# sdwyc/ROLO

Hardware: AMD Instinct MI355X
Metric: scans/sec (128k-pt frame, 20 GN iters) (higher is better)
Workload: dtype f64

## Files before the change

### rolo_amd/csrc/dev_math.hpp

```cpp
#pragma once
#include <hip/hip_runtime.h>

#define ROLO_DEV __device__ __forceinline__

namespace rolo {

ROLO_DEV int f2ord(float f) { int i = __float_as_int(f); return i >= 0 ? i : i ^ 0x7fffffff; }
ROLO_DEV float ord2f(int k) { int i = k >= 0 ? k : k ^ 0x7fffffff; return __int_as_float(i); }


struct Sym3 { double xx, xy, xz, yy, yz, zz; };
struct Vec3 { double x, y, z; };
struct Mat3 { double m[9]; };

ROLO_DEV Vec3 mat3_mulv(const double* R, const Vec3& p) {
  return Vec3{R[0] * p.x + R[1] * p.y + R[2] * p.z, R[3] * p.x + R[4] * p.y + R[5] * p.z, R[6] * p.x + R[7] * p.y + R[8] * p.z};
}

ROLO_DEV Sym3 sym3_rotate(const double* R, const Sym3& C) {
  double a00 = R[0] * C.xx + R[1] * C.xy + R[2] * C.xz, a01 = R[0] * C.xy + R[1] * C.yy + R[2] * C.yz, a02 = R[0] * C.xz + R[1] * C.yz + R[2] * C.zz;
  double a10 = R[3] * C.xx + R[4] * C.xy + R[5] * C.xz, a11 = R[3] * C.xy + R[4] * C.yy + R[5] * C.yz, a12 = R[3] * C.xz + R[4] * C.yz + R[5] * C.zz;
  double a20 = R[6] * C.xx + R[7] * C.xy + R[8] * C.xz, a21 = R[6] * C.xy + R[7] * C.yy + R[8] * C.yz, a22 = R[6] * C.xz + R[7] * C.yz + R[8] * C.zz;
  Sym3 o;
  o.xx = a00 * R[0] + a01 * R[1] + a02 * R[2];
  o.xy = a00 * R[3] + a01 * R[4] + a02 * R[5];
  o.xz = a00 * R[6] + a01 * R[7] + a02 * R[8];
  o.yy = a10 * R[3] + a11 * R[4] + a12 * R[5];
  o.yz = a10 * R[6] + a11 * R[7] + a12 * R[8];
  o.zz = a20 * R[6] + a21 * R[7] + a22 * R[8];
  return o;
}

ROLO_DEV Sym3 sym3_add(const Sym3& a, const Sym3& b) { return Sym3{a.xx + b.xx, a.xy + b.xy, a.xz + b.xz, a.yy + b.yy, a.yz + b.yz, a.zz + b.zz}; }

ROLO_DEV Sym3 sym3_inverse(const Sym3& A) {
  double c00 = A.yy * A.zz - A.yz * A.yz;
  double c01 = A.xz * A.yz - A.xy * A.zz;
  double c02 = A.xy * A.yz - A.xz * A.yy;
  double c11 = A.xx * A.zz - A.xz * A.xz;
  double c12 = A.xz * A.xy - A.xx * A.yz;
  double c22 = A.xx * A.yy - A.xy * A.xy;
  double det = A.xx * c00 + A.xy * c01 + A.xz * c02;
  double inv = 1.0 / det;
  return Sym3{c00 * inv, c01 * inv, c02 * inv, c11 * inv, c12 * inv, c22 * inv};
}

ROLO_DEV Vec3 sym3_mulv(const Sym3& M, const Vec3& e) {
  return Vec3{M.xx * e.x + M.xy * e.y + M.xz * e.z, M.xy * e.x + M.yy * e.y + M.yz * e.z, M.xz * e.x + M.yz * e.y + M.zz * e.z};
}
ROLO_DEV double dot3(const Vec3& a, const Vec3& b) { return a.x * b.x + a.y * b.y + a.z * b.z; }

template <int OFF>
ROLO_DEV int lane_xor_b32(int x) {
  if constexpr (OFF == 32) {
    const auto r = __builtin_amdgcn_permlane32_swap((unsigned)x, (unsigned)x, false, false);
    return (int)((threadIdx.x & 32) ? r[0] : r[1]);
  } else if constexpr (OFF == 16) {
    const auto r = __builtin_amdgcn_permlane16_swap((unsigned)x, (unsigned)x, false, false);
    return (int)((threadIdx.x & 16) ? r[0] : r[1]);
  } else if constexpr (OFF == 8) {
    return __builtin_amdgcn_update_dpp(0, x, 0x128, 0xf, 0xf, false);
  } else if constexpr (OFF == 4) {
    const int a = __builtin_amdgcn_update_dpp(0, x, 0x104, 0xf, 0x5, false);
    return __builtin_amdgcn_update_dpp(a, x, 0x114, 0xf, 0xa, false);
  } else if constexpr (OFF == 2) {
    return __builtin_amdgcn_update_dpp(0, x, 0x4E, 0xf, 0xf, false);
  } else {
    return __builtin_amdgcn_update_dpp(0, x, 0xB1, 0xf, 0xf, false);
  }
}
template <int OFF>
ROLO_DEV double lane_xor_f64(double v) {
  return __hiloint2double(lane_xor_b32<OFF>(__double2hiint(v)), lane_xor_b32<OFF>(__double2loint(v)));
}

template <int OFF>
ROLO_DEV unsigned long long lane_xor_u64(unsigned long long v) {
  const unsigned lo = (unsigned)lane_xor_b32<OFF>((int)(unsigned)(v & 0xffffffffull)), hi = (unsigned)lane_xor_b32<OFF>((int)(unsigned)(v >> 32));
  return ((unsigned long long)hi << 32) | lo;
}

}
```

### rolo_amd/csrc/knn_cov.hip

```cpp
#include <cstdio>
#include <cstring>
#include <string.h>
#include "rolo_internal.hpp"
#include "switches.hpp"
#include "dev_math.hpp"
#include "voxel_dev.hpp"
#ifdef ROLO_KNN_ROCPRIM_SORT
#include <rocprim/rocprim.hpp>
#endif
#include <cfloat>
#include <climits>

namespace rolo {

namespace {


constexpr int BBOX_BLOCKS = 128;
constexpr int BBOX_PART = 16;

__global__ __launch_bounds__(256) void bbox_kernel(KnnPair A, int* bbox) {
  __shared__ float smn[4][3], smx[4][3];
  const int which = blockIdx.x / BBOX_BLOCKS, blk = blockIdx.x - which * BBOX_BLOCKS;
  const float4* __restrict__ p = A.c[which].xyz;
// ... 263 lines not shown
  if (g < P && s < n) {
    const uint32_t idx = order[s];
    const float4 q = p[idx];
    o = make_float4(q.x, q.y, q.z, __int_as_float((int)idx));
  }
  if (g >= P) return;
  const bool real = __float_as_int(o.w) != INT_MAX;
  float lox = real ? o.x : INFINITY, loy = real ? o.y : INFINITY, loz = real ? o.z : INFINITY;
  float hix = real ? o.x : -INFINITY, hiy = real ? o.y : -INFINITY, hiz = real ? o.z : -INFINITY;
  if (g < n_leaves) sorted[s] = o;
#pragma unroll
  for (int m = 1; m < KNN_LEAF; m <<= 1) {
    lox = fminf(lox, __shfl_xor(lox, m)); loy = fminf(loy, __shfl_xor(loy, m)); loz = fminf(loz, __shfl_xor(loz, m));
    hix = fmaxf(hix, __shfl_xor(hix, m)); hiy = fmaxf(hiy, __shfl_xor(hiy, m)); hiz = fmaxf(hiz, __shfl_xor(hiz, m));
  }
  if ((s & (KNN_LEAF - 1)) == 0) {
    boxes[2 * (size_t)(P + g)] = make_float4(lox, loy, loz, 0.f);
    boxes[2 * (size_t)(P + g) + 1] = make_float4(hix, hiy, hiz, 0.f);
  }
  constexpr int LPB = 256 / KNN_LEAF;
  if (P >= LPB) {
    __shared__ float4 nlo[LPB], nhi[LPB];
    const int lt = threadIdx.x / KNN_LEAF;
    if ((s & (KNN_LEAF - 1)) == 0) { nlo[lt] = make_float4(lox, loy, loz, 0.f); nhi[lt] = make_float4(hix, hiy, hiz, 0.f); }
    __syncthreads();
    const size_t g0 = (size_t)P + (size_t)(g - lt);
    int m = LPB; size_t first = g0;
    while (m > 1) {
      const int half = m >> 1;
      first >>= 1;
      float4 a, b;
      const int u = threadIdx.x;
      if (u < half) {
        const float4 l0 = nlo[2 * u], l1 = nlo[2 * u + 1], h0 = nhi[2 * u], h1 = nhi[2 * u + 1];
        a = make_float4(fminf(l0.x, l1.x), fminf(l0.y, l1.y), fminf(l0.z, l1.z), 0.f);
        b = make_float4(fmaxf(h0.x, h1.x), fmaxf(h0.y, h1.y), fmaxf(h0.z, h1.z), 0.f);
      }
      __syncthreads();
      if (u < half) { nlo[u] = a; nhi[u] = b; boxes[2 * (first + u)] = a; boxes[2 * (first + u) + 1] = b; }
      __syncthreads();
      m = half;
    }
  }
}

__global__ __launch_bounds__(256) void tree_reduce_kernel(float4* boxes0, int count_in0, int chunk0, int split, float4* boxes1, int count_in1, int chunk1) {
  ROLO_ALL_KERNEL_PRIO();
  __shared__ float4 lo[512], hi[512];
  const bool second = (int)blockIdx.x >= split;
  float4* boxes = second ? boxes1 : boxes0;
  const int count_in = second ? count_in1 : count_in0, chunk = second ? chunk1 : chunk0;
  const int b = (int)blockIdx.x - (second ? split : 0), t = threadIdx.x;
  const size_t base_in = (size_t)count_in + (size_t)b * chunk;
  for (int i = t; i < chunk; i += 256) { lo[i] = boxes[2 * (base_in + i)]; hi[i] = boxes[2 * (base_in + i) + 1]; }
  __syncthreads();
  int m = chunk, level_count = count_in;
  while (m > 1) {
    const int half = m >> 1;
    level_count >>= 1;
    float4 nlo, nhi;
    if (t < half) {
      float4 a = lo[2 * t], c = lo[2 * t + 1], e = hi[2 * t], f = hi[2 * t + 1];
      nlo = make_float4(fminf(a.x, c.x), fminf(a.y, c.y), fminf(a.z, c.z), 0.f);
      nhi = make_float4(fmaxf(e.x, f.x), fmaxf(e.y, f.y), fmaxf(e.z, f.z), 0.f);
    }
    __syncthreads();
    if (t < half) {
      lo[t] = nlo; hi[t] = nhi;
      size_t h = (size_t)level_count + (size_t)b * half + t;
      boxes[2 * h] = nlo; boxes[2 * h + 1] = nhi;
    }
    __syncthreads();
    m = half;
  }
}

struct Rot2 { double c, s; };

ROLO_DEV void make_jacobi(double x, double y, double z, Rot2& r) {
  double deno = 2.0 * fabs(y);
  if (deno < DBL_MIN) { r.c = 1; r.s = 0; return; }
  double tau = (x - z) / deno;
  double w = sqrt(tau * tau + 1.0);
  double t = (tau > 0) ? 1.0 / (tau + w) : 1.0 / (tau - w);
  double sign_t = t > 0 ? 1.0 : -1.0;
  double n = 1.0 / sqrt(t * t + 1.0);
  r.s = -sign_t * (y / fabs(y)) * fabs(t) * n;
  r.c = n;
}

template <int P_, int Q_>
ROLO_DEV bool jacobi_pair(double (&W)[9], double (&U)[9], double (&V)[9], double& max_diag) {
  const double threshold = fmax(DBL_MIN, 2.0 * DBL_EPSILON * max_diag);
  if (!(fabs(W[P_ * 3 + Q_]) > threshold || fabs(W[Q_ * 3 + P_]) > threshold)) return false;
  double m00 = W[P_ * 3 + P_], m01 = W[P_ * 3 + Q_], m10 = W[Q_ * 3 + P_], m11 = W[Q_ * 3 + Q_];
  Rot2 rot1;
  double t = m00 + m11, d = m10 - m01;
  if (fabs(d) < DBL_MIN) { rot1.s = 0; rot1.c = 1; }
  else { double u = t / d; double tmp = sqrt(1.0 + u * u); rot1.s = 1.0 / tmp; rot1.c = u / tmp; }
  double n00 = rot1.c * m00 + rot1.s * m10, n01 = rot1.c * m01 + rot1.s * m11, n11 = -rot1.s * m01 + rot1.c * m11;
  Rot2 jr; make_jacobi(n00, n01, n11, jr);
  Rot2 jl; { double c2 = jr.c, s2 = -jr.s; jl.c = rot1.c * c2 - rot1.s * s2; jl.s = rot1.c * s2 + rot1.s * c2; }
#pragma unroll
  for (int k = 0; k < 3; k++) { double x = W[P_ * 3 + k], y = W[Q_ * 3 + k]; W[P_ * 3 + k] = jl.c * x + jl.s * y; W[Q_ * 3 + k] = -jl.s * x + jl.c * y; }
#pragma unroll
  for (int k = 0; k < 3; k++) { double x = U[k * 3 + P_], y = U[k * 3 + Q_]; U[k * 3 + P_] = jl.c * x + jl.s * y; U[k * 3 + Q_] = -jl.s * x + jl.c * y; }
#pragma unroll
  for (int k = 0; k < 3; k++) { double x = W[k * 3 + P_], y = W[k * 3 + Q_]; W[k * 3 + P_] = jr.c * x - jr.s * y; W[k * 3 + Q_] = jr.s * x + jr.c * y; }
#pragma unroll
  for (int k = 0; k < 3; k++) { double x = V[k * 3 + P_], y = V[k * 3 + Q_]; V[k * 3 + P_] = jr.c * x - jr.s * y; V[k * 3 + Q_] = jr.s * x + jr.c * y; }
  max_diag = fmax(max_diag, fmax(fabs(W[P_ * 3 + P_]), fabs(W[Q_ * 3 + Q_])));
  return true;
}

ROLO_DEV void swap_cols(double (&M)[9], int a, int b) {
#pragma unroll
  for (int k = 0; k < 3; k++) { double t = M[k * 3 + a]; M[k * 3 + a] = M[k * 3 + b]; M[k * 3 + b] = t; }
}

ROLO_DEV void jacobi_svd3(const double (&A)[9], double (&U)[9], double (&sv)[3], double (&V)[9]) {
  double scale = 0;
#pragma unroll
  for (int i = 0; i < 9; i++) scale = fmax(scale, fabs(A[i]));
  if (!(scale > 0) || !isfinite(scale)) scale = 1.0;
  double W[9];
#pragma unroll
  for (int i = 0; i < 9; i++) { W[i] = A[i] / scale; U[i] = (i % 4 == 0) ? 1.0 : 0.0; V[i] = (i % 4 == 0) ? 1.0 : 0.0; }
  double max_diag = fmax(fabs(W[0]), fmax(fabs(W[4]), fabs(W[8])));
  for (int sweep = 0; sweep < 100; sweep++) {
    bool any = false;
    any |= jacobi_pair<1, 0>(W, U, V, max_diag);
    any |= jacobi_pair<2, 0>(W, U, V, max_diag);
    any |= jacobi_pair<2, 1>(W, U, V, max_diag);
    if (!any) break;
  }
#pragma unroll
  for (int i = 0; i < 3; i++) {
    double a = fabs(W[i * 4]);
    sv[i] = a * scale;
    if (a != 0) { double sgn = W[i * 4] / a; U[0 * 3 + i] *= sgn; U[1 * 3 + i] *= sgn; U[2 * 3 + i] *= sgn; }
  }
  if (sv[1] > sv[0] && sv[1] >= sv[2]) { double t = sv[0]; sv[0] = sv[1]; sv[1] = t; swap_cols(U, 0, 1); swap_cols(V, 0, 1); }
  else if (sv[2] > sv[0] && sv[2] > sv[1]) { double t = sv[0]; sv[0] = sv[2]; sv[2] = t; swap_cols(U, 0, 2); swap_cols(V, 0, 2); }
  if (sv[2] > sv[1]) { double t = sv[1]; sv[1] = sv[2]; sv[2] = t; swap_cols(U, 1, 2); swap_cols(V, 1, 2); }
}

ROLO_DEV void inv3(const double (&A)[9], double (&o)[9]) {
  double c00 = A[4] * A[8] - A[5] * A[7], c01 = A[2] * A[7] - A[1] * A[8], c02 = A[1] * A[5] - A[2] * A[4];
  double c10 = A[5] * A[6] - A[3] * A[8], c11 = A[0] * A[8] - A[2] * A[6], c12 = A[2] * A[3] - A[0] * A[5];
  double c20 = A[3] * A[7] - A[4] * A[6], c21 = A[1] * A[6] - A[0] * A[7], c22 = A[0] * A[4] - A[1] * A[3];
  double det = A[0] * c00 + A[1] * c10 + A[2] * c20;
  double inv = 1.0 / det;
  o[0] = c00 * inv; o[1] = c01 * inv; o[2] = c02 * inv; o[3] = c10 * inv; o[4] = c11 * inv; o[5] = c12 * inv; o[6] = c20 * inv; o[7] = c21 * inv; o[8] = c22 * inv;
}

ROLO_DEV void knn_covariance_finish(double cxx, double cxy, double cxz, double cyy, double cyz, double czz, int n, int qi, int reg,
                                    double* __restrict__ cov, double (&c6)[6], double* __restrict__ nrm = nullptr) {
  double out[9];

  if (reg == ROLO_REG_NONE) {
    out[0] = cxx; out[1] = cxy; out[2] = cxz; out[3] = cxy; out[4] = cyy; out[5] = cyz; out[6] = cxz; out[7] = cyz; out[8] = czz;
  } else if (reg == ROLO_REG_FROBENIUS) {
    double C[9] = {cxx + 1e-3, cxy, cxz, cxy, cyy + 1e-3, cyz, cxz, cyz, czz + 1e-3};
    double Ci[9]; inv3(C, Ci);
    double nrm = 0;
#pragma unroll
    for (int i = 0; i < 9; i++) nrm += Ci[i] * Ci[i];
    nrm = sqrt(nrm);
#pragma unroll
    for (int i = 0; i < 9; i++) Ci[i] /= nrm;
    inv3(Ci, out);
  } else {
    const double A[9] = {cxx, cxy, cxz, cxy, cyy, cyz, cxz, cyz, czz};
    double U[9], V[9], sv[3];
    jacobi_svd3(A, U, sv, V);
    double v0 = 1, v1 = 1, v2 = 1e-3;
    if (reg == ROLO_REG_MIN_EIG) { v0 = fmax(sv[0], 1e-3); v1 = fmax(sv[1], 1e-3); v2 = fmax(sv[2], 1e-3); }
    else if (reg == ROLO_REG_NORMALIZED_MIN_EIG) { double m = fmax(sv[0], fmax(sv[1], sv[2])); v0 = fmax(sv[0] / m, 1e-3); v1 = fmax(sv[1] / m, 1e-3); v2 = fmax(sv[2] / m, 1e-3); }
    else if (reg == ROLO_REG_PLANE_S) { double s = sv[0] + sv[1] + sv[2]; v0 = sv[0] / s; v1 = sv[1] / s; v2 = 1e-3; }
#pragma unroll
    for (int a = 0; a < 3; a++)
#pragma unroll
      for (int b = 0; b < 3; b++) out[a * 3 + b] = (U[a * 3 + 0] * v0) * V[b * 3 + 0] + (U[a * 3 + 1] * v1) * V[b * 3 + 1] + (U[a * 3 + 2] * v2) * V[b * 3 + 2];
    if (nrm && reg == ROLO_REG_PLANE) {
      const double s3 = U[0 * 3 + 2] * V[0 * 3 + 2] + U[1 * 3 + 2] * V[1 * 3 + 2] + U[2 * 3 + 2] * V[2 * 3 + 2];
      const double al = sqrt(1.0 - (s3 < 0 ? -1e-3 : 1e-3));
      const double s1 = U[0 * 3 + 0] * V[0 * 3 + 0] + U[1 * 3 + 0] * V[1 * 3 + 0] + U[2 * 3 + 0] * V[2 * 3 + 0];
      const double s2 = U[0 * 3 + 1] * V[0 * 3 + 1] + U[1 * 3 + 1] * V[1 * 3 + 1] + U[2 * 3 + 1] * V[2 * 3 + 1];
      const bool plane_form = s1 > 0 && s2 > 0;
      const size_t pn = (size_t)n;
      nrm[qi] = plane_form ? al * V[0 * 3 + 2] : __builtin_nan(""); nrm[pn + qi] = al * V[1 * 3 + 2]; nrm[2 * pn + qi] = al * V[2 * 3 + 2];
    }
  }
  const size_t pitch = (size_t)n;
  c6[0] = out[0]; c6[1] = 0.5 * (out[1] + out[3]); c6[2] = 0.5 * (out[2] + out[6]); c6[3] = out[4]; c6[4] = 0.5 * (out[5] + out[7]); c6[5] = out[8];
#pragma unroll
  for (int d = 0; d < 6; d++) cov[d * pitch + qi] = c6[d];
}

template <int KMAX>
ROLO_DEV void knn_neighbourhood_moments(const int (&ki)[KMAX], int kk, const float4* __restrict__ orig, double (&m6)[6]) {
  float px[KMAX], py[KMAX], pz[KMAX];
#pragma unroll
  for (int u = 0; u < KMAX; u++) {
    const float4 p = (u < kk) ? orig[ki[u]] : make_float4(0.f, 0.f, 0.f, 0.f);
    px[u] = p.x; py[u] = p.y; pz[u] = p.z;
  }
  double mx = 0, my = 0, mz = 0;
#pragma unroll
  for (int u = 0; u < KMAX; u++) if (u < kk) { mx += (double)px[u]; my += (double)py[u]; mz += (double)pz[u]; }
  mx /= kk; my /= kk; mz /= kk;
  double cxx = 0, cxy = 0, cxz = 0, cyy = 0, cyz = 0, czz = 0;
#pragma unroll
  for (int u = 0; u < KMAX; u++) if (u < kk) {
    const double ax = (double)px[u] - mx, ay = (double)py[u] - my, az = (double)pz[u] - mz;
    cxx += ax * ax; cxy += ax * ay; cxz += ax * az; cyy += ay * ay; cyz += ay * az; czz += az * az;
  }
  m6[0] = cxx / kk; m6[1] = cxy / kk; m6[2] = cxz / kk; m6[3] = cyy / kk; m6[4] = cyz / kk; m6[5] = czz / kk;
}

template <int KMAX>
ROLO_DEV void knn_covariance_tail(const int (&ki)[KMAX], int kk, const float4* __restrict__ orig, int n, int qi, int reg,
                                  double* __restrict__ cov, double (&c6)[6], double* __restrict__ nrm = nullptr) {
// ... 27 lines not shown
#ifdef ROLO_KNN_ROCPRIM_SORT
  return false;
#else
  return true;
#endif
}

size_t knn_bbox_ints() { return BBOX_PART + 2 * BBOX_BLOCKS * 6; }

size_t knn_sort_temp_bytes(int n) {
#ifdef ROLO_KNN_ROCPRIM_SORT
  size_t bytes = 0;
  (void)rocprim::radix_sort_pairs(nullptr, bytes, (uint32_t*)nullptr, (uint32_t*)nullptr, (uint32_t*)nullptr, (uint32_t*)nullptr,
                                  (size_t)n, 0, 31, (hipStream_t)0);
  return bytes;
#else
  (void)n;
  return sizeof(int) * SORT_PASSES * SORT_NB * SORT_D;
#endif
}

hipError_t launch_knn_build(const KnnPair& A_in, void* sort_tmp, size_t sort_tmp_bytes, uint32_t* keys0, uint32_t* keys1,
                            uint32_t* vals0, uint32_t* vals1, int* bbox, const VoxelFuse& vf, hipStream_t s) {
  KnnPair A = A_in;
  bool have_parts = true;
  for (int i = 0; i < A.n_clouds; i++) have_parts = have_parts && A.c[i].bpart != nullptr && A.c[i].n_bpart > 0;
  if (!have_parts) for (int i = 0; i < A.n_clouds; i++) { A.c[i].bpart = bbox + BBOX_PART + i * BBOX_BLOCKS * 6; A.c[i].n_bpart = BBOX_BLOCKS; }
  const int nc = A.n_clouds;
  const int n_total = A.c[0].n + (nc > 1 ? A.c[1].n : 0);
#ifdef ROLO_KNN_ROCPRIM_SORT
  const int tile_ = ((n_total + SORT_NB - 1) / SORT_NB + SORT_T - 1) / SORT_T * SORT_T;
  if (!have_parts) bbox_kernel<<<BBOX_BLOCKS * nc, 256, 0, s>>>(A, bbox);
  morton_kernel<<<SORT_NB + (vf.enabled ? VF_CLEAR_BLOCKS : 0), SORT_T, 0, s>>>(A, bbox, keys0, vals0, n_total, tile_, nullptr, vf);
  hipError_t e = rocprim::radix_sort_pairs(sort_tmp, sort_tmp_bytes, keys0, keys1, vals0, vals1, (size_t)n_total, 0, nc > 1 ? KEY_BITS : KEY_BITS - 1, s);
  if (e != hipSuccess) return e;
  const uint32_t* order = vals1;
#else
  (void)sort_tmp_bytes;
  int* cnt = static_cast<int*>(sort_tmp);
  const int gvf = vf.enabled ? ((vf.n_tgt + SORT_PASSES - 1) / SORT_PASSES + SORT_T - 1) / SORT_T : 0;
  const int tile = ((n_total + SORT_NB - 1) / SORT_NB + SORT_T - 1) / SORT_T * SORT_T;
  if (!have_parts) bbox_kernel<<<BBOX_BLOCKS * nc, 256, 0, s>>>(A, bbox);
  morton_kernel<<<SORT_NB + (vf.enabled ? VF_CLEAR_BLOCKS : 0), SORT_T, 0, s>>>(A, bbox, keys0, vals0, n_total, tile, cnt, vf);
  uint32_t *ki = keys0, *vi = vals0, *ko = keys1, *vo = vals1;
  for (int p = 0; p < SORT_PASSES; p++) {
    if (p > 0) sort_hist_kernel<<<SORT_NB, SORT_T, 0, s>>>(ki, n_total, tile, p, cnt);
    sort_scatter_kernel<<<SORT_NB + gvf, SORT_T, 0, s>>>(ki, vi, ko, vo, n_total, tile, p, cnt, vf);
    uint32_t* t1 = ki; ki = ko; ko = t1; t1 = vi; vi = vo; vo = t1;
  }
  const uint32_t* order = vi;
#endif
  static_assert(256 % KNN_LEAF == 0 && (KNN_LEAF & (KNN_LEAF - 1)) == 0, "leaf_kernel reduces a leaf inside a wavefront");
  const int l0 = (A.c[0].P * KNN_LEAF + 255) / 256, l1 = nc > 1 ? (A.c[1].P * KNN_LEAF + 255) / 256 : 0;
  leaf_kernel<<<l0 + l1, 256, 0, s>>>(A, l0, order);
  constexpr int LPB = 256 / KNN_LEAF;
  int count0 = A.c[0].P >= LPB ? A.c[0].P / LPB : A.c[0].P, count1 = nc > 1 ? (A.c[1].P >= LPB ? A.c[1].P / LPB : A.c[1].P) : 1;
  while (count0 > 1 || count1 > 1) {
    const int chunk0 = count0 < 512 ? count0 : 512, chunk1 = count1 < 512 ? count1 : 512;
    const int b0 = count0 > 1 ? count0 / chunk0 : 0, b1 = count1 > 1 ? count1 / chunk1 : 0;
    tree_reduce_kernel<<<b0 + b1, 256, 0, s>>>(A.c[0].boxes, count0, chunk0, b0, nc > 1 ? A.c[1].boxes : nullptr, count1, chunk1);
    if (count0 > 1) count0 /= chunk0;
    if (count1 > 1) count1 /= chunk1;
  }
  return hipGetLastError();
}

#ifdef ROLO_KNN_STATS
extern "C" int rolo_debug_wave_records(unsigned* out ) {
  (void)hipDeviceSynchronize();
  return hipMemcpyFromSymbol(out, HIP_SYMBOL(g_knn_wave_rec), sizeof(unsigned) * 16384 * 8) == hipSuccess ? 0 : -1;
}
#endif

static inline int slice_blocks(const KnnCloud& c) { return (c.q_end - c.q_begin + 255) / 256; }

constexpr int KNN_SUB_MAX_PACKETS = 1792;
hipError_t launch_knn_walk(const KnnPair& A, int k, hipStream_t s, int* lanes_out, bool device_busy, bool moments) {
  if (lanes_out) *lanes_out = 1;
  constexpr int QPB = 256;
  const int n0 = A.c[0].q_end - A.c[0].q_begin, n1 = A.n_clouds > 1 ? A.c[1].q_end - A.c[1].q_begin : 0;
  const int g0 = (n0 + QPB - 1) / QPB, g1 = (n1 + QPB - 1) / QPB;
  if (g0 + g1 == 0) return hipSuccess;
  for (int i = 0; i < A.n_clouds; i++) if (A.c[i].q_end > A.c[i].q_begin && A.c[i].q_begin % 64 != 0) return hipErrorInvalidValue;
  if (k > 64) {
    KnnPair R = A;
    for (int r = 0; 64 * r < k; r++) {
      const int kr = k - 64 * r < 64 ? k - 64 * r : 64;
      for (int i = 0; i < R.n_clouds; i++) { R.c[i].slot0 = 64 * r; R.c[i].k_total = k; }
      if (r == 0) knn_walk_kernel<64><<<g0 + g1, 256, 0, s>>>(R, g0, kr);
      else knn_walk_kernel<64, true><<<g0 + g1, 256, 0, s>>>(R, g0, kr);
    }
    return hipGetLastError();
  }
  if (k == 20) {
    const int sub_env = switches().knn_sub;
    const int packets = (n0 + 63) / 64 + (n1 + 63) / 64;
    const int lanes = sub_env < 0 ? (packets <= KNN_SUB_MAX_PACKETS ? 4 : (device_busy ? 0 : 2)) : (sub_env == 2 ? 2 : (sub_env ? 4 : 0));
    if (lanes_out) *lanes_out = lanes ? lanes : 1;
    if (lanes == 4) { const int s0 = (n0 + 63) / 64, s1 = (n1 + 63) / 64; if (moments) knn_walk_sub_kernel<4, true><<<s0 + s1, 256, 0, s>>>(A, s0); else knn_walk_sub_kernel<4><<<s0 + s1, 256, 0, s>>>(A, s0); }
    else if (lanes == 2) { const int s0 = (n0 + 127) / 128, s1 = (n1 + 127) / 128; if (moments) knn_walk_sub_kernel<2, true><<<s0 + s1, 256, 0, s>>>(A, s0); else knn_walk_sub_kernel<2><<<s0 + s1, 256, 0, s>>>(A, s0); }
    else if (moments) knn_walk_kernel<20, false, true><<<g0 + g1, 256, 0, s>>>(A, g0, k);
    else knn_walk_kernel<20><<<g0 + g1, 256, 0, s>>>(A, g0, k);
  }
  else if (k > 32) knn_walk_kernel<64><<<g0 + g1, 256, 0, s>>>(A, g0, k);
  else knn_walk_kernel<32><<<g0 + g1, 256, 0, s>>>(A, g0, k);
  return hipGetLastError();
}

hipError_t launch_knn_unstage(const KnnPair& A, bool own_slice_only, const VoxelFuse& vf, hipStream_t s) {
  const int g0 = own_slice_only ? slice_blocks(A.c[0]) : (A.c[0].n_sorted + 255) / 256;
  const int g1 = A.n_clouds > 1 ? (own_slice_only ? slice_blocks(A.c[1]) : (A.c[1].n_sorted + 255) / 256) : 0;
  if (g0 + g1 == 0) return hipSuccess;
  VoxelFuse v = vf;
  if (own_slice_only) v.enabled = 0;
  knn_unstage_kernel<<<g0 + g1, 256, 0, s>>>(A, g0, own_slice_only ? 1 : 0, v);
  return hipGetLastError();
}

hipError_t launch_knn_tail(const KnnPair& A, int k, int regularization, const VoxelFuse& vf, hipStream_t s, bool moments) {
  const int g0 = slice_blocks(A.c[0]), g1 = A.n_clouds > 1 ? slice_blocks(A.c[1]) : 0;
  if (g0 + g1 == 0) return hipSuccess;
  if (k > 64) knn_tail_loop_kernel<<<g0 + g1, 256, 0, s>>>(A, g0, k, regularization, vf);
  else if (k == 20 && moments) knn_tail_kernel<20, true><<<g0 + g1, 256, 0, s>>>(A, g0, k, regularization, vf);
  else if (k == 20) knn_tail_kernel<20><<<g0 + g1, 256, 0, s>>>(A, g0, k, regularization, vf);
  else if (k <= 32) knn_tail_kernel<32><<<g0 + g1, 256, 0, s>>>(A, g0, k, regularization, vf);
  else knn_tail_kernel<64><<<g0 + g1, 256, 0, s>>>(A, g0, k, regularization, vf);
  return hipGetLastError();
}

}
```

### rolo_amd/csrc/knn_packet.hpp

```cpp
#pragma once
#include "rolo_internal.hpp"
#include "dev_math.hpp"
#include "knn_seed_net.hpp"
#include "knn_box_pair.hpp"
#include <cfloat>
#include <climits>

#ifndef KNN_STAT
#ifdef ROLO_KNN_STATS
#define KNN_STAT(x) x
#else
#define KNN_STAT(x)
#endif
#endif

namespace rolo {
namespace {

constexpr int WALK_STACK = KNN_WALK_STACK;

ROLO_DEV double key_pack(float d2, int idx) {
  return __longlong_as_double((long long)(((unsigned long long)__float_as_uint(d2) << 32) | (unsigned)idx));
}
ROLO_DEV float key_d2(double k) { return __uint_as_float((unsigned)((unsigned long long)__double_as_longlong(k) >> 32)); }
// ... 7 lines not shown
ROLO_DEV void insert_slot(double& ks, double ksm1, double c) { ks = vmax_f64(ksm1, vmin_f64(c, ks)); }
#endif
#ifndef ROLO_KNN_B1
#define ROLO_KNN_B1 15
#define ROLO_KNN_B2 10
#define ROLO_KNN_B3 5
#endif
template <int KMAX>
ROLO_DEV void insert_tiered(double (&K)[KMAX], double ck) {
  constexpr int B1 = KMAX == 20 ? ROLO_KNN_B1 : 3 * (KMAX / 4), B2 = KMAX == 20 ? ROLO_KNN_B2 : 2 * (KMAX / 4), B3 = KMAX == 20 ? ROLO_KNN_B3 : KMAX / 4;
#pragma unroll
  for (int s = KMAX - 1; s >= B1; s--) insert_slot(K[s], K[s - 1], ck);
  if (__any(ck < K[B1 - 1])) {
#pragma unroll
    for (int s = B1 - 1; s >= B2; s--) insert_slot(K[s], K[s - 1], ck);
    if (__any(ck < K[B2 - 1])) {
#pragma unroll
      for (int s = B2 - 1; s >= B3; s--) insert_slot(K[s], K[s - 1], ck);
      if (__any(ck < K[B3 - 1])) {
#pragma unroll
        for (int s = B3 - 1; s >= 1; s--) insert_slot(K[s], K[s - 1], ck);
        K[0] = vmin_f64(ck, K[0]);
      }
    }
  }
}

ROLO_DEV void sload_leaf(const float4* __restrict__ p, float4 (&pts)[KNN_LEAF]) {
#pragma unroll
  for (int u = 0; u < KNN_LEAF; u++) pts[u] = p[u];
}
ROLO_DEV void sload_node(const float4* __restrict__ p, float4& llo, float4& lhi, float4& rlo, float4& rhi) { llo = p[0]; lhi = p[1]; rlo = p[2]; rhi = p[3]; }

template <int KMAX, bool LOWER> constexpr bool walk_bound_in_list() { return KMAX == 20 && !LOWER; }

template <int KMAX, bool LOWER = false>
ROLO_DEV void knn_score_leaf(const float4* __restrict__ sorted, int g, const float4& q, double (&K)[KMAX], int kk, double& bkey, float& bd,
                             unsigned& n_ins, unsigned& lane_acc, unsigned& rounds, double lo = 0.0) {
  float4 pts[KNN_LEAF];
  sload_leaf(sorted + KNN_LEAF * (size_t)g, pts);
  constexpr bool IN_LIST = walk_bound_in_list<KMAX, LOWER>();
  KNN_STAT(const double bkey0 = IN_LIST ? K[KMAX - 1] : bkey; unsigned my_acc = 0;)
#ifdef ROLO_KNN_STATS2
  unsigned my_cur = 0;
#endif
#pragma unroll
  for (int u = 0; u < KNN_LEAF; u++) {
    const float4 c = pts[u];
    const float dx = q.x - c.x, dy = q.y - c.y, dz = q.z - c.z;
    const float cd = ((dx * dx) + (dy * dy)) + (dz * dz);
    const double ck0 = key_pack(cd, __float_as_int(c.w));
    const double ck = (LOWER && !(ck0 > lo)) ? key_pack(INFINITY, INT_MAX) : ck0;
    const bool better = IN_LIST ? ck < K[KMAX - 1] : ck < bkey;
    KNN_STAT(if (__any(better)) { n_ins++; lane_acc += (unsigned)__popcll(__ballot(better)); })
    KNN_STAT(if (ck < bkey0) my_acc++;)
#ifdef ROLO_KNN_STATS2
    if (better) my_cur++;
#endif
    if (better) {
      insert_tiered<KMAX>(K, ck);
      if constexpr (!IN_LIST) {
#pragma unroll
        for (int s = 0; s < KMAX; s++) if (s == kk - 1) bkey = K[s];
        bd = key_d2(bkey);
      }
    }
  }
#ifdef ROLO_KNN_STATS
#ifdef ROLO_KNN_STATS2
  rounds += my_cur;
  (void)my_acc;
#else
  { unsigned m = my_acc;
    for (int off = 32; off > 0; off >>= 1) m = max(m, (unsigned)__shfl_xor((int)m, off, 64));
    rounds += m; }
#endif
#endif
}

struct KeyMin { ROLO_DEV double operator()(double a, double b) const { return vmin_f64(a, b); } };
struct KeyMax { ROLO_DEV double operator()(double a, double b) const { return vmax_f64(a, b); } };

template <int NB, int STRIDE, class P>
ROLO_DEV void seed_chunk(const P& p, int first, const float4& q, double (&K)[20]) {
  double b[NB];
#pragma unroll
  for (int u = 0; u < NB; u++) {
    const float4 c = p[first + u * STRIDE];
    const float dx = q.x - c.x, dy = q.y - c.y, dz = q.z - c.z;
    const float cd = ((dx * dx) + (dy * dy)) + (dz * dz);
    b[u] = key_pack(cd, __float_as_int(c.w));
  }
  if constexpr (NB == 8) seednet::sort8(b, KeyMin(), KeyMax()); else seednet::sort4(b, KeyMin(), KeyMax());
  seednet::merge_chunk<NB>(K, b, KeyMin(), KeyMax());
}

ROLO_DEV void knn_seed_leaf(const float4* __restrict__ sorted, int g, const float4& q, double (&K)[20]) {
  static_assert(KNN_LEAF == 16, "two chunks of 8");
  float4 pts[KNN_LEAF];
  sload_leaf(sorted + KNN_LEAF * (size_t)g, pts);
  seed_chunk<8, 1>(pts, 0, q, K);
  seed_chunk<8, 1>(pts, 8, q, K);
}

template <int CTRL>
ROLO_DEV double dpp_f64(double x) {
  const long long v = __double_as_longlong(x);
  const int lo = __builtin_amdgcn_mov_dpp((int)(unsigned)(unsigned long long)v, CTRL, 0xF, 0xF, true);
  const int hi = __builtin_amdgcn_mov_dpp((int)(unsigned)((unsigned long long)v >> 32), CTRL, 0xF, 0xF, true);
  return __longlong_as_double((long long)(((unsigned long long)(unsigned)hi << 32) | (unsigned)lo));
}
template <int ST> ROLO_DEV double sub_xchg(double x) { return ST == 0 ? dpp_f64<0xB1>(x) : ST == 1 ? dpp_f64<0x4E>(x) : dpp_f64<0x141>(x); }
template <int SUB> ROLO_DEV double sub_min(double x) {
  x = vmin_f64(x, sub_xchg<0>(x));
  if (SUB >= 4) x = vmin_f64(x, sub_xchg<1>(x));
  if (SUB >= 8) x = vmin_f64(x, sub_xchg<2>(x));
  return x;
}
template <int SUB> ROLO_DEV double sub_max(double x) {
  x = vmax_f64(x, sub_xchg<0>(x));
  if (SUB >= 4) x = vmax_f64(x, sub_xchg<1>(x));
  if (SUB >= 8) x = vmax_f64(x, sub_xchg<2>(x));
  return x;
}

ROLO_DEV int xcd_contiguous_block(int b, int G, int wpb = 4) {
#ifdef ROLO_KNN_NO_XCD_REMAP
  return b;
#else
  if (G * wpb <= 2048) {
    const int x = b & 7, k = b >> 3, q = G >> 3, r = G & 7;
    return x * q + min(x, r) + k;
  }
  const int RUN = 256 / wpb, GROUP = 8 * RUN;
  if (b >= G / GROUP * GROUP) return b;
  const int grp = b / GROUP, o = b - grp * GROUP;
  return grp * GROUP + (o & 7) * RUN + (o >> 3);
#endif
}

typedef __attribute__((address_space(3))) int lds_int;

template <int KMAX, bool LOWER>
ROLO_DEV void packet_walk(const float4* __restrict__ sorted, const float4* __restrict__ boxes, int P, int g_own0, int g_own1, const float4& q, double (&K)[KMAX], int kk,
                          double& bkey, float& bd, double lo, lds_int* stk, int& sp, int h,
                          unsigned& st_nodes, unsigned& st_leaves, unsigned& st_ins, unsigned& st_lane, unsigned& st_rounds, unsigned& st_push) {
  (void)st_push;
  while (true) {
    h = __builtin_amdgcn_readfirstlane(h);
    if (h < P) {
      st_nodes++;
      float4 llo, lhi, rlo, rhi;
      sload_node(boxes + 4 * (size_t)h, llo, lhi, rlo, rhi);
      const box_f2 d = box_d2_pair(llo, lhi, rlo, rhi, q);
      const float bl = d[0], br = d[1], bdc = box_bound_clamp(walk_bound_in_list<KMAX, LOWER>() ? key_d2(K[KMAX - 1]) : bd);
      const bool okl = box_reached(bl, bdc), okr = box_reached(br, bdc);
      const unsigned long long ml = __ballot(okl), mr = __ballot(okr);
      if (ml != 0ull && mr != 0ull) {
        const unsigned long long pref = __ballot((okl || okr) && (bl <= br));
        const bool left_first = 2 * __popcll(pref) >= __popcll(ml | mr);
        if (sp < WALK_STACK) { stk[sp] = left_first ? 2 * h + 1 : 2 * h; sp++; KNN_STAT(st_push++;) }
        h = left_first ? 2 * h : 2 * h + 1;
        continue;
      }
      if (ml != 0ull) { h = 2 * h; continue; }
      if (mr != 0ull) { h = 2 * h + 1; continue; }
    } else {
      const int g = h - P;
      if (g < g_own0 || g >= g_own1) {
        knn_score_leaf<KMAX, LOWER>(sorted, g, q, K, kk, bkey, bd, st_ins, st_lane, st_rounds, lo);
        st_leaves++;
      }
    }
    if (sp == 0) return;
    sp--;
    h = stk[sp];
  }
}

template <int KMAX, bool LOWER>
ROLO_DEV void packet_climb(const float4* __restrict__ sorted, const float4* __restrict__ boxes, int P, int g_mine0, int g_own0, int g_own1, const float4& q, double (&K)[KMAX], int kk,
                           double& bkey, float& bd, double lo, lds_int* stk,
                           unsigned& st_nodes, unsigned& st_leaves, unsigned& st_ins, unsigned& st_lane, unsigned& st_rounds, unsigned& st_push) {
  for (int a = (P + g_mine0) >> 2; a > 1; a >>= 1) {
    const int s = a ^ 1;
// ... 15 lines not shown
```

### rolo_amd/csrc/knn_seed_net.hpp

```cpp
#pragma once

#if defined(__HIPCC__) || defined(__CUDACC__)
#define ROLO_NET_FN __host__ __device__ __forceinline__
#define ROLO_NET_UNROLL _Pragma("unroll")
#else
#define ROLO_NET_FN inline
#define ROLO_NET_UNROLL
#endif

namespace rolo {
namespace seednet {

template <class T, class Min, class Max>
ROLO_NET_FN void cx(T& a, T& b, Min mn, Max mx) {
  const T lo = mn(a, b);
  b = mx(a, b);
  a = lo;
}

template <class T, class Min, class Max>
ROLO_NET_FN void sort8(T (&b)[8], Min mn, Max mx) {
  constexpr int net[19][2] = {{0, 2}, {1, 3}, {4, 6}, {5, 7}, {0, 4}, {1, 5}, {2, 6}, {3, 7}, {0, 1}, {2, 3}, {4, 5}, {6, 7}, {2, 4}, {3, 5}, {1, 4}, {3, 6}, {1, 2}, {3, 4}, {5, 6}};
ROLO_NET_UNROLL
  for (int c = 0; c < 19; c++) cx(b[net[c][0]], b[net[c][1]], mn, mx);
}

template <class T, class Min, class Max>
ROLO_NET_FN void sort4(T (&b)[4], Min mn, Max mx) {
  cx(b[0], b[1], mn, mx); cx(b[2], b[3], mn, mx); cx(b[0], b[2], mn, mx); cx(b[1], b[3], mn, mx); cx(b[1], b[2], mn, mx);
}

template <int N, int OFF, bool DESC, class T, int KN, class Min, class Max>
ROLO_NET_FN void bitonic_clean(T (&K)[KN], Min mn, Max mx) {
  constexpr int P2 = N <= 4 ? 4 : N <= 8 ? 8 : N <= 16 ? 16 : 32, PAD = P2 - N;
  static_assert(N <= 32 && OFF + N <= KN, "run inside the list");
ROLO_NET_UNROLL
  for (int d = P2 / 2; d >= 1; d >>= 1) {
ROLO_NET_UNROLL
    for (int p = PAD; p < P2; p++) {
      if ((p & d) == 0) {
        if (DESC) cx(K[OFF + p + d - PAD], K[OFF + p - PAD], mn, mx);
        else cx(K[OFF + p - PAD], K[OFF + p + d - PAD], mn, mx);
      }
    }
  }
}

template <int NB, class T, class Min, class Max>
ROLO_NET_FN void merge_chunk(T (&K)[20], const T (&b)[NB], Min mn, Max mx) {
  static_assert(NB == 8 || NB == 4, "chunk size");
ROLO_NET_UNROLL
  for (int i = 0; i < NB; i++) K[20 - NB + i] = mn(K[20 - NB + i], b[NB - 1 - i]);
  bitonic_clean<NB, 20 - NB, true>(K, mn, mx);
  bitonic_clean<20, 0, false>(K, mn, mx);
}
template <class T, class Min, class Max>
ROLO_NET_FN void merge8(T (&K)[20], const T (&b)[8], Min mn, Max mx) { merge_chunk<8>(K, b, mn, mx); }

}
}
```

### rolo_amd/csrc/knn_walk.hpp

```cpp
#pragma once
#ifdef ROLO_KNN_STATS
#define KNN_STAT(x) x
#else
#define KNN_STAT(x)
#endif
#include "knn_packet.hpp"

namespace rolo {
namespace {

ROLO_DEV double* stage_area(const KnnCloud& cl, unsigned add) {
  double* s = cl.stage;
  if (cl.stage_epoch) {
    const unsigned long long e = __hip_atomic_load(cl.stage_epoch, __ATOMIC_RELAXED, __HIP_MEMORY_SCOPE_SYSTEM) + add;
    if (e & 1ull) s += cl.stage_alt;
  }
  return s;
}

#ifdef ROLO_KNN_STATS
__device__ unsigned g_knn_wave_rec[16384][8];
#endif

template <int KMAX>
ROLO_DEV void walk_write_lists(const KnnCloud& cl, const double (&K)[KMAX], int kk, double bkey, int qi, int j) {
  int ki[KMAX];
#pragma unroll
  for (int u = 0; u < KMAX; u++) ki[u] = key_idx(K[u]);
  const int slot0 = (KMAX == 64) ? cl.slot0 : 0;
  const int ktot = (KMAX == 64 && cl.k_total) ? cl.k_total : kk;
  if (cl.knn_idx) {
#pragma unroll
    for (int u = 0; u < KMAX; u++) if (u < kk) { cl.knn_idx[(size_t)qi * ktot + slot0 + u] = ki[u]; cl.knn_d2[(size_t)qi * ktot + slot0 + u] = key_d2(K[u]); }
  }
  if (KMAX == 64 && cl.lower) cl.lower[j] = bkey;
  int32_t* __restrict__ nbr = cl.nbr;
#pragma unroll
  for (int u = 0; u < KMAX; u++) nbr[(size_t)(slot0 + u) * cl.n_sorted + j] = ki[u];
}

template <int KMAX>
ROLO_DEV void walk_write_moments(const KnnCloud& cl, const double (&K)[KMAX], int kk, int qi, int j, int (*s_ki)[256]) {
  if (cl.knn_idx) {
#pragma unroll
    for (int u = 0; u < KMAX; u++) if (u < kk) { cl.knn_idx[(size_t)qi * kk + u] = key_idx(K[u]); cl.knn_d2[(size_t)qi * kk + u] = key_d2(K[u]); }
  }
  const int tid = threadIdx.x;
#pragma unroll
  for (int u = 0; u < KMAX; u++) s_ki[u][tid] = key_idx(K[u]);
  const float4* __restrict__ orig = cl.xyz;
  double mx = 0, my = 0, mz = 0;
#pragma unroll 5
  for (int u = 0; u < kk; u++) { const float4 p = orig[s_ki[u][tid]]; mx += (double)p.x; my += (double)p.y; mz += (double)p.z; }
  mx /= kk; my /= kk; mz /= kk;
  double cxx = 0, cxy = 0, cxz = 0, cyy = 0, cyz = 0, czz = 0;
#pragma unroll 5
  for (int u = 0; u < kk; u++) {
    const float4 p = orig[s_ki[u][tid]];
    const double ax = (double)p.x - mx, ay = (double)p.y - my, az = (double)p.z - mz;
    cxx += ax * ax; cxy += ax * ay; cxz += ax * az; cyy += ay * ay; cyz += ay * az; czz += az * az;
  }
  double* __restrict__ mom = reinterpret_cast<double*>(cl.nbr);
  const size_t pitch = (size_t)cl.n_sorted;
  mom[j] = cxx / kk; mom[pitch + j] = cxy / kk; mom[2 * pitch + j] = cxz / kk; mom[3 * pitch + j] = cyy / kk; mom[4 * pitch + j] = cyz / kk; mom[5 * pitch + j] = czz / kk;
}

#ifndef ROLO_KNN_WALK_OCC
#define ROLO_KNN_WALK_OCC 4
#endif
#ifndef ROLO_KNN_PACKET
#define ROLO_KNN_PACKET 64
#endif
#ifndef ROLO_KNN_SEED_EXTRA
#define ROLO_KNN_SEED_EXTRA 1
#endif
static_assert(ROLO_KNN_PACKET == 64, "one query per lane");

template <int KMAX, bool LOWER>
ROLO_DEV void walk_seeds(const float4* __restrict__ sorted, int g_mine0, int g_own0, int g_own1, int n_leaves, const float4& q, bool active, double (&K)[KMAX], int kk, double& bkey, float& bd, double lo,
                         unsigned& st_leaves, unsigned& st_ins, unsigned& st_lane, unsigned& st_rounds) {
  const int n_own = min(g_mine0 + 64 / KNN_LEAF, n_leaves) - g_mine0, n_before = g_mine0 - g_own0;
  for (int i = 0; i < g_own1 - g_own0; i++) {
    const int g = i < n_own ? g_mine0 + i : (i - n_own < n_before ? g_own0 + (i - n_own) : g_mine0 + (i - n_before));
    if constexpr (KMAX == 20 && !LOWER) knn_seed_leaf(sorted, g, q, K);
    else knn_score_leaf<KMAX, LOWER>(sorted, g, q, K, kk, bkey, bd, st_ins, st_lane, st_rounds, lo);
    st_leaves++;
  }
  if constexpr (KMAX == 20 && !LOWER) {
    if (!active) {
#pragma unroll
      for (int u = 0; u < KMAX; u++) K[u] = key_pack(0.f, 0);
    }
  }
}

template <int KMAX, bool LOWER = false, bool MOMENTS = false>
__global__ __launch_bounds__(256, KMAX > 32 ? 2 : (MOMENTS ? 6 : ROLO_KNN_WALK_OCC)) void knn_walk_kernel(KnnPair A, int split, int k) {
  __shared__ int stk[4][WALK_STACK];
  __shared__ int s_ki[MOMENTS ? KMAX : 1][256];
  const int tid = threadIdx.x;
  const int wv = tid >> 6;
  const int blk = xcd_contiguous_block((int)blockIdx.x, (int)gridDim.x, 4);
  const int which = blk >= split ? 1 : 0;
  const float4* __restrict__ sorted = A.c[which].sorted;
  const float4* __restrict__ boxes = A.c[which].boxes;
  const int n_sorted = A.c[which].n_sorted, P = A.c[which].P;
  const int lane_ = tid & 63;
  const int j = A.c[which].q_begin + (blk - (which ? split : 0)) * 256 + wv * 64 + lane_;
  float4 q = make_float4(INFINITY, INFINITY, INFINITY, 0.f);
  int qi = INT_MAX;
  if (j < A.c[which].q_end) { q = sorted[j]; qi = __float_as_int(q.w); }
  const bool active = qi != INT_MAX;
  const int kk = (KMAX == 20) ? 20 : k;
  const int n_leaves = n_sorted / KNN_LEAF;
  unsigned st_nodes = 0, st_leaves = 0, st_ins = 0, st_lane = 0, st_rounds = 0, st_push = 0;

  const double sentinel = key_pack(INFINITY, INT_MAX);
  double K[KMAX];
#pragma unroll
  for (int u = 0; u < KMAX; u++) K[u] = sentinel;
  float bd = active ? INFINITY : -1.0f;
  double bkey = active ? sentinel : key_pack(0.f, 0);

  const int g_mine0 = __builtin_amdgcn_readfirstlane(j / KNN_LEAF);
  const int g_own0 = max(g_mine0 - ROLO_KNN_SEED_EXTRA, 0);
  const int g_own1 = min(g_mine0 + 64 / KNN_LEAF + ROLO_KNN_SEED_EXTRA, n_leaves);
  double lo = 0.0;
  if (LOWER && active) lo = A.c[which].lower[j];
  (void)lo;
  walk_seeds<KMAX, LOWER>(sorted, g_mine0, g_own0, g_own1, n_leaves, q, active, K, kk, bkey, bd, lo, st_leaves, st_ins, st_lane, st_rounds);

  int g_climb = g_mine0;
#ifdef ROLO_KNN_STATS
  unsigned long long wt0;
  { int zero; asm("s_memrealtime %0\n\ts_waitcnt lgkmcnt(0)\n\ts_mov_b32 %1, 0" : "=s"(wt0), "=s"(zero)); g_climb += zero; }
#endif
  if (g_mine0 < n_leaves)
    packet_climb<KMAX, LOWER>(sorted, boxes, P, g_climb, g_own0, g_own1, q, K, kk, bkey, bd, lo, (lds_int*)&stk[wv][0], st_nodes, st_leaves, st_ins, st_lane, st_rounds, st_push);
#ifdef ROLO_KNN_STATS
  { unsigned long long wt1; asm volatile("s_memrealtime %0\n\ts_waitcnt lgkmcnt(0)" : "=s"(wt1));
    unsigned st_rounds_rec = st_rounds;
#ifdef ROLO_KNN_STATS2
    for (int off = 32; off > 0; off >>= 1) st_rounds_rec = max(st_rounds_rec, (unsigned)__shfl_xor((int)st_rounds_rec, off, 64));
#endif
    const unsigned wid = blockIdx.x * 4 + (threadIdx.x >> 6);
    if ((threadIdx.x & 63) == 0 && wid < 16384) {
      g_knn_wave_rec[wid][0] = st_nodes; g_knn_wave_rec[wid][1] = st_leaves; g_knn_wave_rec[wid][2] = st_ins; g_knn_wave_rec[wid][3] = st_push;
      g_knn_wave_rec[wid][4] = (unsigned)wt0; g_knn_wave_rec[wid][5] = (unsigned)wt1; g_knn_wave_rec[wid][6] = st_lane; g_knn_wave_rec[wid][7] = st_rounds_rec;
    } }
#endif
  (void)st_nodes; (void)st_leaves; (void)st_ins; (void)st_lane; (void)st_rounds; (void)st_push;

  if (!active) return;

  if (MOMENTS) {
    walk_write_moments<KMAX>(A.c[which], K, kk, qi, j, s_ki);
    return;
  }
  walk_write_lists<KMAX>(A.c[which], K, kk, bkey, qi, j);
}

template <int ST> ROLO_DEV void merge20(double (&K)[20]) {
#pragma unroll
  for (int j = 0; j < 10; j++) {
    const double o1 = sub_xchg<ST>(K[19 - j]), o2 = sub_xchg<ST>(K[j]);
    K[j] = vmin_f64(K[j], o1);
    K[19 - j] = vmin_f64(K[19 - j], o2);
// ... 253 lines not shown
```

Measured before the change: 5119.

## Trim divisions, dead comparators and address math in kNN covariance kernels

Replaces several f64 divisions with one shared reciprocal plus Newton/FMA refinement, guarded by range checks that fall back to true division. Sign flips in the Jacobi/SVD code now use bit manipulation and copysign instead of divisions. The seed merge network skips comparators known to be dead, and the first leaf is merged with a 16-element bitonic cleaner instead of two full 20-element merges. Point gathers use unsigned 32-bit byte offsets, and a new point-count limit is checked on the host to keep that safe. These cut ALU work in the kNN walk and moments code, but the guarded paths add wave-level votes and branches, and rounding may differ slightly from true division.

```diff
diff --git a/rolo_amd/csrc/dev_math.hpp b/rolo_amd/csrc/dev_math.hpp
--- a/rolo_amd/csrc/dev_math.hpp
+++ b/rolo_amd/csrc/dev_math.hpp
@@ -8,6 +8,19 @@
 ROLO_DEV int f2ord(float f) { int i = __float_as_int(f); return i >= 0 ? i : i ^ 0x7fffffff; }
 ROLO_DEV float ord2f(int k) { int i = k >= 0 ? k : k ^ 0x7fffffff; return __int_as_float(i); }
 
+
+ROLO_DEV double div_den(double b) {
+  double y = __builtin_amdgcn_rcp(b);
+  double f = __builtin_fma(-b, y, 1.0);
+  y = __builtin_fma(y, f, y);
+  f = __builtin_fma(-b, y, 1.0);
+  return __builtin_fma(y, f, y);
+}
+ROLO_DEV double div_shared(double a, double b, double y) {
+  const double q = a * y;
+  return __builtin_fma(__builtin_fma(-b, q, a), y, q);
+}
+ROLO_DEV bool div_shared_ok(double v) { return fabs(v) >= 0x1p-500 && fabs(v) <= 0x1p500; }
 
 struct Sym3 { double xx, xy, xz, yy, yz, zz; };
 struct Vec3 { double x, y, z; };
diff --git a/rolo_amd/csrc/knn_cov.hip b/rolo_amd/csrc/knn_cov.hip
--- a/rolo_amd/csrc/knn_cov.hip
+++ b/rolo_amd/csrc/knn_cov.hip
@@ -369,10 +369,11 @@
   if (deno < DBL_MIN) { r.c = 1; r.s = 0; return; }
   double tau = (x - z) / deno;
   double w = sqrt(tau * tau + 1.0);
-  double t = (tau > 0) ? 1.0 / (tau + w) : 1.0 / (tau - w);
-  double sign_t = t > 0 ? 1.0 : -1.0;
+  double t = 1.0 / ((tau > 0) ? tau + w : tau - w);
   double n = 1.0 / sqrt(t * t + 1.0);
-  r.s = -sign_t * (y / fabs(y)) * fabs(t) * n;
+  const double mag = fabs(t) * n + fabs(y) * 0.0;
+  const int flip = ((t > 0) ? (int)0x80000000 : 0) ^ (__double2hiint(y) & (int)0x80000000);
+  r.s = __hiloint2double(__double2hiint(mag) ^ flip, __double2loint(mag));
   r.c = n;
 }
 
@@ -384,7 +385,11 @@
   Rot2 rot1;
   double t = m00 + m11, d = m10 - m01;
   if (fabs(d) < DBL_MIN) { rot1.s = 0; rot1.c = 1; }
-  else { double u = t / d; double tmp = sqrt(1.0 + u * u); rot1.s = 1.0 / tmp; rot1.c = u / tmp; }
+  else {
+    double u = t / d; double tmp = sqrt(1.0 + u * u);
+    if (fabs(u) >= 0x1p-500 && tmp <= 0x1p499) { const double rt = div_den(tmp); rot1.s = div_shared(1.0, tmp, rt); rot1.c = div_shared(u, tmp, rt); }
+    else { rot1.s = 1.0 / tmp; rot1.c = u / tmp; }
+  }
   double n00 = rot1.c * m00 + rot1.s * m10, n01 = rot1.c * m01 + rot1.s * m11, n11 = -rot1.s * m01 + rot1.c * m11;
   Rot2 jr; make_jacobi(n00, n01, n11, jr);
   Rot2 jl; { double c2 = jr.c, s2 = -jr.s; jl.c = rot1.c * c2 - rot1.s * s2; jl.s = rot1.c * s2 + rot1.s * c2; }
@@ -425,7 +430,7 @@
   for (int i = 0; i < 3; i++) {
     double a = fabs(W[i * 4]);
     sv[i] = a * scale;
-    if (a != 0) { double sgn = W[i * 4] / a; U[0 * 3 + i] *= sgn; U[1 * 3 + i] *= sgn; U[2 * 3 + i] *= sgn; }
+    if (a != 0) { double sgn = copysign(1.0, W[i * 4]) + W[i * 4] * 0.0; U[0 * 3 + i] *= sgn; U[1 * 3 + i] *= sgn; U[2 * 3 + i] *= sgn; }
   }
   if (sv[1] > sv[0] && sv[1] >= sv[2]) { double t = sv[0]; sv[0] = sv[1]; sv[1] = t; swap_cols(U, 0, 1); swap_cols(V, 0, 1); }
   else if (sv[2] > sv[0] && sv[2] > sv[1]) { double t = sv[0]; sv[0] = sv[2]; sv[2] = t; swap_cols(U, 0, 2); swap_cols(V, 0, 2); }
@@ -619,6 +624,7 @@
   const int g0 = (n0 + QPB - 1) / QPB, g1 = (n1 + QPB - 1) / QPB;
   if (g0 + g1 == 0) return hipSuccess;
   for (int i = 0; i < A.n_clouds; i++) if (A.c[i].q_end > A.c[i].q_begin && A.c[i].q_begin % 64 != 0) return hipErrorInvalidValue;
+  for (int i = 0; i < A.n_clouds; i++) if (A.c[i].n >= KNN_MAX_POINTS) return hipErrorInvalidValue;
   if (k > 64) {
     KnnPair R = A;
     for (int r = 0; 64 * r < k; r++) {
diff --git a/rolo_amd/csrc/knn_packet.hpp b/rolo_amd/csrc/knn_packet.hpp
--- a/rolo_amd/csrc/knn_packet.hpp
+++ b/rolo_amd/csrc/knn_packet.hpp
@@ -113,8 +113,7 @@
 struct KeyMax { ROLO_DEV double operator()(double a, double b) const { return vmax_f64(a, b); } };
 
 template <int NB, int STRIDE, class P>
-ROLO_DEV void seed_chunk(const P& p, int first, const float4& q, double (&K)[20]) {
-  double b[NB];
+ROLO_DEV void seed_keys(const P& p, int first, const float4& q, double (&b)[NB]) {
 #pragma unroll
   for (int u = 0; u < NB; u++) {
     const float4 c = p[first + u * STRIDE];
@@ -123,15 +122,28 @@
     b[u] = key_pack(cd, __float_as_int(c.w));
   }
   if constexpr (NB == 8) seednet::sort8(b, KeyMin(), KeyMax()); else seednet::sort4(b, KeyMin(), KeyMax());
+}
+template <int NB, int STRIDE, class P>
+ROLO_DEV void seed_chunk(const P& p, int first, const float4& q, double (&K)[20]) {
+  double b[NB];
+  seed_keys<NB, STRIDE>(p, first, q, b);
   seednet::merge_chunk<NB>(K, b, KeyMin(), KeyMax());
 }
 
+template <bool FIRST>
 ROLO_DEV void knn_seed_leaf(const float4* __restrict__ sorted, int g, const float4& q, double (&K)[20]) {
   static_assert(KNN_LEAF == 16, "two chunks of 8");
   float4 pts[KNN_LEAF];
   sload_leaf(sorted + KNN_LEAF * (size_t)g, pts);
-  seed_chunk<8, 1>(pts, 0, q, K);
-  seed_chunk<8, 1>(pts, 8, q, K);
+  if constexpr (FIRST) {
+    double b0[8], b1[8];
+    seed_keys<8, 1>(pts, 0, q, b0);
+    seed_keys<8, 1>(pts, 8, q, b1);
+    seednet::first_two_chunks(K, b0, b1, KeyMin(), KeyMax());
+  } else {
+    seed_chunk<8, 1>(pts, 0, q, K);
+    seed_chunk<8, 1>(pts, 8, q, K);
+  }
 }
 
 template <int CTRL>
diff --git a/rolo_amd/csrc/knn_seed_net.hpp b/rolo_amd/csrc/knn_seed_net.hpp
--- a/rolo_amd/csrc/knn_seed_net.hpp
+++ b/rolo_amd/csrc/knn_seed_net.hpp
@@ -30,29 +30,38 @@
   cx(b[0], b[1], mn, mx); cx(b[2], b[3], mn, mx); cx(b[0], b[2], mn, mx); cx(b[1], b[3], mn, mx); cx(b[1], b[2], mn, mx);
 }
 
-template <int N, int OFF, bool DESC, class T, int KN, class Min, class Max>
-ROLO_NET_FN void bitonic_clean(T (&K)[KN], Min mn, Max mx) {
+template <int N, int OFF, bool DESC, int ASC, class T, int KN, class Min, class Max>
+ROLO_NET_FN void bitonic_clean_known(T (&K)[KN], Min mn, Max mx) {
   constexpr int P2 = N <= 4 ? 4 : N <= 8 ? 8 : N <= 16 ? 16 : 32, PAD = P2 - N;
   static_assert(N <= 32 && OFF + N <= KN, "run inside the list");
+  static_assert(ASC == 0 || (!DESC && N == 20), "the dead comparators are worked out for the ascending 20-cleaner");
 ROLO_NET_UNROLL
   for (int d = P2 / 2; d >= 1; d >>= 1) {
 ROLO_NET_UNROLL
     for (int p = PAD; p < P2; p++) {
       if ((p & d) == 0) {
+        if (d == 8 && p - PAD >= 4 && p + d - PAD < ASC) continue;
         if (DESC) cx(K[OFF + p + d - PAD], K[OFF + p - PAD], mn, mx);
         else cx(K[OFF + p - PAD], K[OFF + p + d - PAD], mn, mx);
       }
     }
   }
 }
+template <int N, int OFF, bool DESC, class T, int KN, class Min, class Max>
+ROLO_NET_FN void bitonic_clean(T (&K)[KN], Min mn, Max mx) { bitonic_clean_known<N, OFF, DESC, 0>(K, mn, mx); }
 
 template <int NB, class T, class Min, class Max>
 ROLO_NET_FN void merge_chunk(T (&K)[20], const T (&b)[NB], Min mn, Max mx) {
   static_assert(NB == 8 || NB == 4, "chunk size");
 ROLO_NET_UNROLL
   for (int i = 0; i < NB; i++) K[20 - NB + i] = mn(K[20 - NB + i], b[NB - 1 - i]);
-  bitonic_clean<NB, 20 - NB, true>(K, mn, mx);
-  bitonic_clean<20, 0, false>(K, mn, mx);
+  bitonic_clean_known<20, 0, false, 20 - NB>(K, mn, mx);
+}
+template <class T, class Min, class Max>
+ROLO_NET_FN void first_two_chunks(T (&K)[20], const T (&b0)[8], const T (&b1)[8], Min mn, Max mx) {
+ROLO_NET_UNROLL
+  for (int i = 0; i < 8; i++) { K[i] = b0[i]; K[8 + i] = b1[7 - i]; }
+  bitonic_clean<16, 0, false>(K, mn, mx);
 }
 template <class T, class Min, class Max>
 ROLO_NET_FN void merge8(T (&K)[20], const T (&b)[8], Min mn, Max mx) { merge_chunk<8>(K, b, mn, mx); }
diff --git a/rolo_amd/csrc/knn_walk.hpp b/rolo_amd/csrc/knn_walk.hpp
--- a/rolo_amd/csrc/knn_walk.hpp
+++ b/rolo_amd/csrc/knn_walk.hpp
@@ -39,6 +39,11 @@
   for (int u = 0; u < KMAX; u++) nbr[(size_t)(slot0 + u) * cl.n_sorted + j] = ki[u];
 }
 
+constexpr int KNN_MAX_POINTS = 1 << 28;
+ROLO_DEV float4 gather_point(const float4* __restrict__ base, int idx) {
+  return *reinterpret_cast<const float4*>(reinterpret_cast<const char*>(base) + ((unsigned)idx << 4));
+}
+
 template <int KMAX>
 ROLO_DEV void walk_write_moments(const KnnCloud& cl, const double (&K)[KMAX], int kk, int qi, int j, int (*s_ki)[256]) {
   if (cl.knn_idx) {
@@ -51,18 +56,26 @@
   const float4* __restrict__ orig = cl.xyz;
   double mx = 0, my = 0, mz = 0;
 #pragma unroll 5
-  for (int u = 0; u < kk; u++) { const float4 p = orig[s_ki[u][tid]]; mx += (double)p.x; my += (double)p.y; mz += (double)p.z; }
-  mx /= kk; my /= kk; mz /= kk;
+  for (int u = 0; u < kk; u++) { const float4 p = gather_point(orig, s_ki[u][tid]); mx += (double)p.x; my += (double)p.y; mz += (double)p.z; }
+  const double den = (double)kk, rden = div_den(den);
+  if (!__any(!(div_shared_ok(mx) && div_shared_ok(my) && div_shared_ok(mz)))) { mx = div_shared(mx, den, rden); my = div_shared(my, den, rden); mz = div_shared(mz, den, rden); }
+  else { mx /= kk; my /= kk; mz /= kk; }
   double cxx = 0, cxy = 0, cxz = 0, cyy = 0, cyz = 0, czz = 0;
 #pragma unroll 5
   for (int u = 0; u < kk; u++) {
-    const float4 p = orig[s_ki[u][tid]];
+    const float4 p = gather_point(orig, s_ki[u][tid]);
     const double ax = (double)p.x - mx, ay = (double)p.y - my, az = (double)p.z - mz;
     cxx += ax * ax; cxy += ax * ay; cxz += ax * az; cyy += ay * ay; cyz += ay * az; czz += az * az;
   }
+  if (!__any(!(div_shared_ok(cxx) && div_shared_ok(cxy) && div_shared_ok(cxz) && div_shared_ok(cyy) && div_shared_ok(cyz) && div_shared_ok(czz)))) {
+    cxx = div_shared(cxx, den, rden); cxy = div_shared(cxy, den, rden); cxz = div_shared(cxz, den, rden);
+    cyy = div_shared(cyy, den, rden); cyz = div_shared(cyz, den, rden); czz = div_shared(czz, den, rden);
+  } else {
+    cxx /= kk; cxy /= kk; cxz /= kk; cyy /= kk; cyz /= kk; czz /= kk;
+  }
   double* __restrict__ mom = reinterpret_cast<double*>(cl.nbr);
   const size_t pitch = (size_t)cl.n_sorted;
-  mom[j] = cxx / kk; mom[pitch + j] = cxy / kk; mom[2 * pitch + j] = cxz / kk; mom[3 * pitch + j] = cyy / kk; mom[4 * pitch + j] = cyz / kk; mom[5 * pitch + j] = czz / kk;
+  mom[j] = cxx; mom[pitch + j] = cxy; mom[2 * pitch + j] = cxz; mom[3 * pitch + j] = cyy; mom[4 * pitch + j] = cyz; mom[5 * pitch + j] = czz;
 }
 
 #ifndef ROLO_KNN_WALK_OCC
@@ -80,9 +93,13 @@
 ROLO_DEV void walk_seeds(const float4* __restrict__ sorted, int g_mine0, int g_own0, int g_own1, int n_leaves, const float4& q, bool active, double (&K)[KMAX], int kk, double& bkey, float& bd, double lo,
                          unsigned& st_leaves, unsigned& st_ins, unsigned& st_lane, unsigned& st_rounds) {
   const int n_own = min(g_mine0 + 64 / KNN_LEAF, n_leaves) - g_mine0, n_before = g_mine0 - g_own0;
-  for (int i = 0; i < g_own1 - g_own0; i++) {
+  int i = 0;
+  if constexpr (KMAX == 20 && !LOWER) {
+    if (g_own1 - g_own0 > 0) { knn_seed_leaf<true>(sorted, n_own > 0 ? g_mine0 : g_own0, q, K); st_leaves++; i = 1; }
+  }
+  for (; i < g_own1 - g_own0; i++) {
     const int g = i < n_own ? g_mine0 + i : (i - n_own < n_before ? g_own0 + (i - n_own) : g_mine0 + (i - n_before));
-    if constexpr (KMAX == 20 && !LOWER) knn_seed_leaf(sorted, g, q, K);
+    if constexpr (KMAX == 20 && !LOWER) knn_seed_leaf<false>(sorted, g, q, K);
     else knn_score_leaf<KMAX, LOWER>(sorted, g, q, K, kk, bkey, bd, st_ins, st_lane, st_rounds, lo);
     st_leaves++;
   }
```

Result: faster. 5209 (median of 6 runs) (+1.8%).
